# pqh22/ProxyTransformation

Hardware: AMD Instinct MI355X
Metric: scenes/sec (100k pts, 256 clusters, 64 proxies) (higher is better)
Workload: dtype f32; 1 GPU; cfg2: N=100000 pts, gs=8->M'=256 kept clusters, L=64 text + V=196 image proxies, d=256, eval forward; scenes_per_gpu=4, img_feat_dtype=bf16, input_sets_rotated=3, streams=1, lanes=1 (one forward at a time), setup_forwards=32

## Files before the change

include/proxyt.h:

```cpp
#ifndef PROXYT_H_
#define PROXYT_H_

#include <stddef.h>
#include <stdint.h>

#ifdef __cplusplus
extern "C" {
#endif

#define PTX_ABI_VERSION 13

#define PTX_API __attribute__((visibility("default")))

#define PTX_OK          0
#define PTX_EINVAL     -1
#define PTX_ELAUNCH    -2
#define PTX_ENOSPACE   -3
#define PTX_ETIMEOUT   -4
#define PTX_EGATE      -5

typedef struct PtxShape {
    int32_t B;
    int32_t N;
    int32_t grid_size;
// ... 54 lines not shown

PTX_API int         ptx_abi_version(void);
PTX_API const char *ptx_last_error(void);

typedef struct PtxContext PtxContext;
PTX_API int ptx_context_create(PtxContext **ctx);
PTX_API int ptx_context_destroy(PtxContext *ctx);
PTX_API int ptx_context_check(PtxContext *ctx);
PTX_API int ptx_context_sync_check(PtxContext *ctx);
PTX_API int ptx_context_gates(const PtxContext *ctx);

PTX_API int         ptx_kernel_count(void);
PTX_API const char *ptx_kernel_name(int kid);
PTX_API int         ptx_timing_select(int kid);
PTX_API int         ptx_timing_read(int *launches, float *total_ms);
PTX_API int         ptx_timing_every(int n);
PTX_API int         ptx_timing_select_mask(uint64_t mask);
PTX_API int         ptx_timing_read_sites(int *launches, float *total_ms, int n);

PTX_API size_t ptx_prep_bytes(const PtxShape *s);
PTX_API size_t ptx_workspace_bytes(const PtxShape *s);

PTX_API int ptx_workspace_init(const PtxShape *s, void *workspace, size_t ws_bytes, void *stream);

PTX_API int ptx_prepare(const PtxShape *s, const PtxWeights *w, const float *lin,
                void *prep, size_t prep_bytes, void *stream);


PTX_API int ptx_grid_centers(const float *points, int B, int N, const float *lin, int gs, float margin,
                     float *minmax, float *centers, void *workspace, size_t ws_bytes, void *stream);

PTX_API int ptx_ball_query(const float *centers, const float *points, int B, int M, int N, int K,
                   float radius, int32_t *idx, float *cluster, int32_t *pad_count, void *stream);

PTX_API int ptx_linear(const float *x, const float *w, const float *bias, const float *residual, float *y,
               int rows, int n_out, int n_in, int gelu, void *stream);
PTX_API int ptx_linear_ln_partials(const float *x, const float *w, const float *bias, const float *residual, float *y, float *lnp,
               int rows, int n_out, int n_in, void *stream);
PTX_API size_t ptx_ln_linear_scratch_bytes(int n_out, int n_in);
PTX_API int ptx_ln_linear(const float *x, const float *lnp, const float *w, const float *gamma, const float *beta,
               const float *bias, float eps, int gelu, float *y, void *scratch, size_t scratch_bytes,
               int rows, int n_out, int n_in, void *stream);
PTX_API int ptx_gemm_policy(int min_tiles_128);

PTX_API int ptx_offset_net(const PtxShape *s, const PtxWeights *w, const void *prep,
                   const float *centers_in, const float *cluster, const float *minmax,
// ... 248 lines not shown
```

proxytransformation_amd/_abi.py:

```python
from __future__ import annotations

import ctypes as C
import os
from typing import Optional

_HERE = os.path.dirname(os.path.abspath(__file__))
LIB_PATH = os.path.join(_HERE, "libproxyt_hip.so")
ABI_VERSION = 13

c_float_p = C.c_void_p


class PtxShape(C.Structure):
    _fields_ = [(n, C.c_int32) for n in
                ("B", "N", "grid_size", "K", "Mt", "Mk", "L", "V", "C", "heads", "hidden",
                 "in_dim", "hw", "img_dtype")] + \
               [(n, C.c_float) for n in ("radius", "margin", "bn_eps", "ln_eps")]


class PtxSlotMlp(C.Structure):
    _fields_ = [(n, C.c_void_p) for n in ("conv_w", "conv_b", "bn_w", "bn_b", "bn_mean", "bn_var")]


class PtxBlock(C.Structure):
# ... 78 lines not shown
                ("arena_bwd", C.c_void_p), ("arena_bwd_bytes", C.c_size_t), ("grads", C.c_void_p), ("grads_floats", C.c_size_t),
                ("dtext", C.c_void_p), ("dimg", C.c_void_p)]


class PtxForwardOpts(C.Structure):
    _fields_ = [("bbox_enc", C.c_void_p), ("compute_dtype", C.c_int32), ("reserved", C.c_int32 * 5)]


_P, _I, _F, _Z = C.c_void_p, C.c_int, C.c_float, C.c_size_t
_SH, _W = C.POINTER(PtxShape), C.POINTER(PtxWeights)
SIGNATURES = {
    "ptx_abi_version": (C.c_int, []),
    "ptx_last_error": (C.c_char_p, []),
    "ptx_kernel_count": (C.c_int, []),
    "ptx_kernel_name": (C.c_char_p, [_I]),
    "ptx_timing_select": (_I, [_I]),
    "ptx_timing_every": (_I, [_I]),
    "ptx_timing_read": (_I, [C.POINTER(C.c_int), C.POINTER(C.c_float)]),
    "ptx_timing_select_mask": (_I, [C.c_uint64]),
    "ptx_timing_read_sites": (_I, [C.POINTER(C.c_int), C.POINTER(C.c_float), _I]),
    "ptx_prep_bytes": (_Z, [_SH]),
    "ptx_workspace_bytes": (_Z, [_SH]),
    "ptx_workspace_init": (_I, [_SH, _P, _Z, _P]),
    "ptx_prepare": (_I, [_SH, _W, _P, _P, _Z, _P]),
    "ptx_grid_centers": (_I, [_P, _I, _I, _P, _I, _F, _P, _P, _P, _Z, _P]),
    "ptx_ball_query": (_I, [_P, _P, _I, _I, _I, _I, _F, _P, _P, _P, _P]),
    "ptx_linear": (_I, [_P, _P, _P, _P, _P, _I, _I, _I, _I, _P]),
    "ptx_linear_ln_partials": (_I, [_P, _P, _P, _P, _P, _P, _I, _I, _I, _P]),
    "ptx_ln_linear_scratch_bytes": (_Z, [_I, _I]),
    "ptx_ln_linear": (_I, [_P, _P, _P, _P, _P, _P, _F, _I, _P, _P, _Z, _I, _I, _I, _P]),
    "ptx_gemm_policy": (_I, [_I]),
    "ptx_offset_net": (_I, [_SH, _W, _P, _P, _P, _P, _P, _P, _P]),
    "ptx_select_clusters": (_I, [_SH] + [_P] * 14),
    "ptx_pointnet": (_I, [_SH, _W, _P, _P, _P, _P, _P]),
    "ptx_img_proxy": (_I, [_SH, _W, _P, _P, _P, _P, _Z, _P]),
    "ptx_proxy_block": (_I, [_SH, _W, _P, _I, _P, _P, _I, _P, _P, _P, _P, _Z, _P]),
    "ptx_affine_scatter": (_I, [_SH, _P, _P, _P, _P, _P, _P, _P]),
    "ptx_affine_compact": (_I, [_SH, _P, _P, _P, _P, _P, _P, _P, _P, _Z, _P]),
    "ptx_wait_counts": (_I, [_P, _I, C.c_int64]),
    "ptx_context_create": (_I, [C.POINTER(C.c_void_p)]),
    "ptx_context_destroy": (_I, [_P]),
    "ptx_context_check": (_I, [_P]),
    "ptx_context_sync_check": (_I, [_P]),
    "ptx_context_gates": (_I, [_P]),
    "ptx_forward": (_I, [_P, _SH, _W, _P, _P, _P, _P, _P, _P, _P, _P, _P, _P, _P, _P, _Z,
                         C.POINTER(PtxDebug), _P]),
# ... 101 lines not shown
```

proxytransformation_amd/csrc/api.hip:

```cpp
#include <atomic>
#include <chrono>
#include <cmath>
#include <cstdlib>
#include <cstring>
#include <mutex>
#include <utility>
#include <vector>

#include "common.h"

namespace ptx {

static thread_local char g_err[512] = "";

void set_error(const char *fmt, ...)
{
    va_list ap;
    va_start(ap, fmt);
    vsnprintf(g_err, sizeof(g_err), fmt, ap);
    va_end(ap);
}

static const char *const kKernelNames[] = {
    "k_minmax", "k_cluster", "k_select", "k_tags",
// ... 99 lines not shown
    P.posb_t = take((size_t)s.Mk * s.C); P.posb_i = take((size_t)s.Mk * s.C);
    P.w3 = take((size_t)3 * s.C * s.in_dim); P.b3 = take((size_t)3 * s.C);
    P.t1 = take((size_t)s.heads * P.KT1 * P.hd);
    P.t2 = take((size_t)s.heads * P.hd * P.KT2p);
    P.ppg_w = take((size_t)s.C * s.C); P.ppg_c = take(s.C);
    for (int i = 0; i < 2; ++i) {
        P.fc1g_w[i] = take((size_t)s.hidden * s.C); P.fc1g_c[i] = take(s.hidden);
        const size_t planes = mlp_fused_supported(s.C, s.hidden, 1, 0) ? (size_t)s.hidden * s.C * 3 / 2 : 0;
        P.mlp_w1p[i] = take(planes); P.mlp_w2p[i] = take(planes);
    }
    for (int i = 0; i < 2; ++i) P.qkvb[i] = take((size_t)s.Mk * 3 * s.C);
    P.total = o;
    return P;
}

struct LayoutForce { int v[4]; };
static LayoutForce layout_force()
{
    LayoutForce f{{-1, -1, -1, -1}};
    if (const char *e = getenv("PTX_LAYOUT"))
        for (int i = 0; i < 4 && e[i] != '\0'; ++i) f.v[i] = e[i] == '0' ? 0 : (e[i] == '1' ? 1 : -1);
    return f;
}
struct LayoutChoice { double est_cluster, est_image; bool cluster_on_caller, img_late, early; LayoutForce lf; };
static LayoutChoice choose_layout(const PtxShape &S)
{
    static const LayoutForce lf = layout_force();
    LayoutChoice c{};
    c.lf = lf;
    const int B = S.B, Kd = S.Mt - S.Mk;
    const double img_mb = (double)B * S.V * S.in_dim * S.hw * (S.img_dtype == 0 ? 4.0 : 2.0) * 1e-6;
    c.est_cluster = 80.0 + 0.42 * Kd;
    c.est_image = 40.0 + (S.img_dtype == 0 ? 0.98 : 0.78) * img_mb;
    c.cluster_on_caller = lf.v[0] >= 0 ? lf.v[0] != 0 : c.est_cluster > c.est_image + 60.0;
    c.img_late = c.cluster_on_caller && (lf.v[2] >= 0 ? lf.v[2] != 0 : c.est_image + 60.0 < 0.8 * c.est_cluster);
    const double est_all = 1.8 * 12.0 * (double)B * S.Mt * S.C * S.C / 70e6;
    c.early = c.cluster_on_caller && (lf.v[1] >= 0 ? lf.v[1] != 0 : (Kd >= 128 && (long)B * S.Mk >= 1024 && est_all < 3.0 * 0.42 * Kd));
    return c;
}

WsLayout ws_layout(const PtxShape &s)
{
    WsLayout L{};
    const PrepLayout P = prep_layout(s);
    size_t o = 0;
    auto take = [&](size_t bytes) { size_t r = o; o += align_up(bytes, 256); return r; };
    const size_t B = s.B, N = s.N, K = s.K, C = s.C;
    const size_t M = (size_t)s.grid_size * s.grid_size * s.grid_size;
    const size_t Mk = s.Mk, Mt = s.Mt, Kd = s.Mt - s.Mk;
    const size_t nimg = B * s.V, Lp = s.L > s.V ? s.L : s.V, R = B * Mk;
    L.zero_begin = o;
    L.mm_enc = take(B * 6 * 4);
    L.scene_acc = take(B * 2 * 4);
    L.tag = take(B * N * 4);
    L.fa_ticket = take(2 * B * s.heads * 4);
    L.mlp_ticket = take(mlp_ticket_bytes((int)R));
    L.mm_ticket = take(4);
    L.zero_bytes = o - L.zero_begin;
    L.minmax = take(B * 6 * 4);
    L.centers0 = take(B * M * 3 * 4); L.cluster1 = take(B * M * K * 3 * 4);
    L.offsets = take(B * M * 3 * 4);  L.centers = take(B * M * 3 * 4);
    L.idx2 = take(B * M * K * 4);     L.cluster2 = take(B * M * K * 3 * 4);
    L.pad_count = take(B * M * 4);
    L.order = take(B * Mt * 4); L.picks = take(B * (Kd ? Kd : 1) * 4); L.keep = take(B * Mk * 4); L.ksrc = take(B * Mk * 4);
    L.kcenter = take(B * Mk * 3 * 4); L.kcluster = take(B * Mk * K * 3 * 4); L.kidx = take(B * Mk * K * 4);
    L.drop_idx = take(B * (Kd ? Kd : 1) * K * 4);
    L.tile_counts = take(B * (size_t)cdiv(s.N, kTilePts) * 4);
    L.point_proxy = take(R * C * 4);
    for (int i = 0; i < 2; ++i) L.x_in[i] = take(R * C * 4);
    bool may_early = false;
    for (int dt = 0; dt < 3; ++dt) { PtxShape t = s; t.img_dtype = dt; may_early = may_early || choose_layout(t).early; }
    const size_t em = may_early ? 1 : 0;
    L.pp_all = take(em * B * Mt * C * 4); L.order_e = take(em * B * Mt * 4);
    for (int i = 0; i < 2; ++i) { L.xln_all[i] = take(em * B * Mt * C * 4); L.g_all[i] = take(em * B * Mt * 3 * C * 4); }
    L.fm = take(nimg * s.in_dim * 4); L.qkv0 = take(nimg * 3 * C * 4);
    L.we = take(nimg * s.heads * (size_t)P.KT1 * 4);
    {
        const size_t pool_b = img_pool_bytes((int)nimg, s.in_dim, P.KT2p - s.in_dim), gbuf_b = nimg * s.heads * (size_t)P.KT2p * 4;
        L.pool = L.gbuf = take(pool_b > gbuf_b ? pool_b : gbuf_b);
    }
    L.obuf = take(nimg * C * 4); L.cbuf = take(nimg * C * 4); L.img_proxy = take(nimg * C * 4);
    for (int i = 0; i < 2; ++i) {
        L.qkv[i] = take(R * 3 * C * 4); L.pt[i] = take(B * Lp * C * 4); L.pv[i] = take(B * Lp * C * 4);
        L.ao[i] = take(R * C * 4); L.x1[i] = take(R * C * 4); L.xn2[i] = take(0);
        L.hbuf[i] = take(mlp_fused_supported(s.C, s.hidden, (int)R, 0) ? 0 : R * (size_t)s.hidden * 4);
        L.x2[i] = take(R * C * 4); L.guide[i] = take(R * C * 4);
        L.head[i] = take(R * 9 * 4);
        L.lnp_x1[i] = take(R * (C / 32) * 2 * 4);
    }
    L.lnp_img = take(nimg * (C / 32) * 2 * 4);
    const size_t fsp = fattn_split_for(s.B, s.heads);
    L.fa_part = take(fsp > 1 ? 2 * B * s.heads * fsp * Mk * kFaPartRow * 4 : 0);
    L.mlp_part = take(mlp_fused_supported(s.C, s.hidden, (int)R, 0) ? mlp_part_bytes((int)R) : 0);
    L.total = o;
    return L;
}

}
struct PtxContext {
    int dev = -1;
    hipStream_t st = nullptr, lo = nullptr;
    hipEvent_t fork = nullptr, join = nullptr, aux = nullptr, tags = nullptr, early_a = nullptr, early_b = nullptr;
    uint32_t *gate = nullptr; uint32_t gate_seq = 0;
// ... 207 lines not shown
            g.p[0].w2 = prep + P.t1; g.p[0].c2 = we; g.p[0].n2 = P.KT1; g.p[0].ldc2 = s.heads * P.KT1;
            g.p[0].chain_tiles = s.heads; g.p[0].w2_stride = (long)P.KT1 * hd; g.p[0].c2_stride = P.KT1;
        }
        PTX_TIMED(KID_IMG_QKV0, st, launch_gemm(g, st));
    }
    if (!chained) {
        for (int h0 = 0; h0 < s.heads; h0 += kMaxGroups) {
            GemmBatch g{}; g.n = std::min(kMaxGroups, s.heads - h0);
            for (int h = h0; h < h0 + g.n; ++h)
                g.p[h - h0] = GemmProb{qkv0 + h * hd, prep + P.t1 + (size_t)h * P.KT1 * hd, we + (size_t)h * P.KT1,
                                       nullptr, nullptr, nullptr, nullptr, nimg, P.KT1, hd, 3 * C, hd,
                                       s.heads * P.KT1, 0, 0, 0, EPI_NONE};
            PTX_TIMED(KID_IMG_WE, st, launch_gemm(g, st));
        }
    }
    if (pooled32) {
        PTX_TIMED_EXT(KID_IMG_SCORES, st, launch_img_pool32(img, we, qkv0, nimg, s.in_dim, s.hw, C, P.KT1, EW, attn_scale(hd), Gs, E, ML, st));
    } else if (dt == 0) {
        PTX_TIMED(KID_IMG_SCORES, st, launch_img_scores(img, we, qkv0, nimg, s.in_dim, s.hw, s.heads, C, P.KT1,
                                                        P.KT2p, attn_scale(hd), gbuf, st));
        PTX_TIMED(KID_IMG_GATHER, st, launch_img_gather(img, nimg, s.in_dim, s.hw, s.heads, P.KT2p, gbuf, st));
    } else if (pooled) {
        PTX_TIMED_EXT(KID_IMG_SCORES, st, launch_img_pool(img_any, dt, we, qkv0, nimg, s.in_dim, s.hw, C, P.KT1,
                                                      EW, attn_scale(hd), Gs, E, ML, st));
    } else {
        PTX_TIMED(KID_IMG_SCORES, st, launch_img_scores16(img_any, dt, we, qkv0, nimg, s.in_dim, s.hw, s.heads, C,
                                                          P.KT1, P.KT2p, attn_scale(hd), gbuf, st));
        PTX_TIMED(KID_IMG_GATHER, st, launch_img_gather16(img_any, dt, nimg, s.in_dim, s.hw, s.heads, P.KT2p, gbuf, st));
    }
    for (int h0 = 0; h0 < s.heads; h0 += kMaxGroups) {
        GemmBatch g{}; g.n = std::min(kMaxGroups, s.heads - h0);
        for (int h = h0; h < h0 + g.n; ++h) {
            GemmProb &gp = g.p[h - h0];
            gp = GemmProb{gbuf + (size_t)h * P.KT2p, prep + P.t2 + (size_t)h * hd * P.KT2p, obuf + h * hd,
                          w.v_b + h * hd, nullptr, gbuf + (size_t)h * P.KT2p + s.in_dim,
                          qkv0 + 2 * C + h * hd, nimg, hd, P.KT2p, s.heads * P.KT2p, P.KT2p, C,
                          0, s.heads * P.KT2p, 3 * C, EPI_NONE};
            if (pooled) {
                gp.A = nullptr; gp.rs = nullptr;
                gp.pg = Gs + (size_t)h * s.in_dim; gp.ldg = 2 * s.heads * s.in_dim; gp.gslab = s.heads * s.in_dim;
                gp.pe = E + (size_t)h * EW; gp.lde = s.heads * EW;
                gp.pml = ML + (size_t)h * 5; gp.ldml = s.heads * 5;
                gp.kg = s.in_dim;
            }
        }
        PTX_TIMED(KID_IMG_O, st, launch_gemm(g, st));
    }
    {
        GemmBatch g{}; g.n = 1;
        g.p[0] = GemmProb{obuf, w.c_w, cbuf, w.c_b, nullptr, nullptr, nullptr,
                          nimg, C, C, C, C, C, 0, 0, 0, EPI_NONE};
        g.p[0].lnp_out = at<float>(ws, L.lnp_img) + (size_t)i0 * (C / 32) * 2;
        PTX_TIMED(KID_IMG_C, st, launch_gemm(g, st));
    }
    if (need_ln) {
        LnBatch lb{}; lb.n = 1; lb.C = C; lb.eps = s.ln_eps;
        lb.p[0] = LnProb{cbuf, img_proxy, w.norm_img_w, w.norm_img_b, nullptr, nimg, 1};
        PTX_TIMED(KID_IMG_LN, st, launch_ln_rows(lb, st));
    }
    return PTX_OK;
}

struct Branch {
    const PtxBlock *blk; const float *x_in; const float *proxy; int Lp; const uint8_t *mask;
    const float *head_w, *head_b, *head_ab; int nout; float *head_out; float *guide; int slot;
    bool late_proxy;
    const float *proxy_lnp, *pp_gw, *pp_gc;
    const float *fc1_gw, *fc1_gc;
// ... 276 lines not shown
            std::chrono::duration_cast<std::chrono::microseconds>(std::chrono::steady_clock::now() - t0).count() >
                timeout_us)
            return PTX_ETIMEOUT;
    }
}

size_t ptx_prep_bytes(const PtxShape *s)
{
    if (s == nullptr || validate_shape(*s) != PTX_OK) return 0;
    return prep_layout(*s).total * sizeof(float);
}

size_t ptx_workspace_bytes(const PtxShape *s)
{
    if (s == nullptr || validate_shape(*s) != PTX_OK) return 0;
    return ws_layout(*s).total;
}

int ptx_workspace_init(const PtxShape *s, void *workspace, size_t ws_bytes, void *stream)
{
    PTX_TRY(check_bufs(s, workspace, ws_bytes));
    const WsLayout L = ws_layout(*s);
    PTX_HIP(hipMemsetAsync(at<char>(workspace, L.zero_begin), 0, L.zero_bytes, static_cast<hipStream_t>(stream)));
    return PTX_OK;
}

int ptx_prepare(const PtxShape *s, const PtxWeights *w, const float *lin, void *prep, size_t prep_bytes,
                void *stream)
{
    (void)lin;
    PTX_REQUIRE(s && w && prep, "ptx_prepare: null argument");
    PTX_TRY(validate_shape(*s));
    if (prep_bytes < prep_layout(*s).total * sizeof(float)) { set_error("prep buffer too small"); return PTX_ENOSPACE; }
    return run_prepare(*s, *w, static_cast<float *>(prep), static_cast<hipStream_t>(stream));
}

int ptx_grid_centers(const float *points, int B, int N, const float *lin, int gs, float margin,
                     float *minmax, float *centers, void *workspace, size_t ws_bytes, void *stream)
{
    PTX_REQUIRE(points && lin && minmax && centers && workspace, "ptx_grid_centers: null argument");
    PTX_REQUIRE(ws_bytes >= (size_t)B * 6 * 4, "ptx_grid_centers: workspace needs %d bytes", B * 24);
    hipStream_t st = static_cast<hipStream_t>(stream);
    uint32_t *enc = static_cast<uint32_t *>(workspace);
    PTX_HIP(hipMemsetAsync(enc, 0, (size_t)B * 6 * 4, st));
    ScenePts sp;
    PTX_TRY(make_scene_pts(points, nullptr, B, N, &sp));
// ... 315 lines not shown
        float *pp_all = at<float>(ws, L.pp_all), *xa_t = at<float>(ws, L.xln_all[0]), *xa_i = at<float>(ws, L.xln_all[1]);
        int32_t *order_e = at<int32_t>(ws, L.order_e);
        PTX_TRY(launch_order(S, pad_count, order_override, order_e, side->lo));
        PTX_TRY(launch_pointnet(pf + P.enc_ab, w->encoder, centers, cluster2, B * S.Mt, S.Mt, K, S.C, pp_all, &w->text, &w->img, nullptr,
                                nullptr, xa_t, xa_i, S.ln_eps, order_e, M, side->lo, nullptr, 0, true));
        GemmBatch g{}; g.n = 2;
        g.p[0] = GemmProb{xa_t, w->text.qkv_w, at<float>(ws, L.g_all[0]), nullptr, nullptr, nullptr, nullptr, B * S.Mt, 3 * S.C, S.C, S.C, S.C,
                          3 * S.C, 0, 0, 0, EPI_NONE};
        g.p[1] = GemmProb{xa_i, w->img.qkv_w, at<float>(ws, L.g_all[1]), nullptr, nullptr, nullptr, nullptr, B * S.Mt, 3 * S.C, S.C, S.C, S.C,
                          3 * S.C, 0, 0, 0, EPI_NONE};
        PTX_TRY(launch_gemm(g, side->lo, compute_dtype));
        PTX_TRY(run_blocks(S, br, 2, point_proxy, ws, side->lo, 1, compute_dtype, nullptr, nullptr, true));
    }

    int32_t *order = at<int32_t>(ws, L.order), *picks = at<int32_t>(ws, L.picks), *keep = at<int32_t>(ws, L.keep);
    float *kcenter = at<float>(ws, L.kcenter);
    float *kcluster = dbg && debug->kcluster ? at<float>(ws, L.kcluster) : nullptr;
    int32_t *kidx = dbg && debug->kidx ? at<int32_t>(ws, L.kidx) : nullptr;
    int32_t *drop_idx = dbg && debug->drop_idx ? at<int32_t>(ws, L.drop_idx) : nullptr;
    int32_t *ksrc = at<int32_t>(ws, L.ksrc);
    const bool ext_event = !capturing;
    const bool tags_gated = gated && side->lo_ok && (lf.v[3] >= 0 ? lf.v[3] != 0 : est_image < 1.6 * est_cluster);
    const bool tags_tail = !cluster_on_caller && !tags_gated;
    PTX_TIMED(KID_SELECT, cs, launch_select_order(S, centers, pad_count, order_override, order, picks, keep, kcenter,
                                                  ksrc, bbox_in ? nullptr : mm_ws, cs, cluster_on_caller, ext_event && !tags_tail ? side->aux : nullptr,
                                                  cg_join_select ? &cjoin : nullptr));
    int32_t *tile_counts = at<int32_t>(ws, L.tile_counts);
    hipStream_t ts = tags_tail ? cs : side->lo;
    const bool slots_first = !cluster_on_caller && !tags_tail;
    auto enqueue_tags = [&]() -> int {
        if (tags_gated) {
            PTX_TIMED(KID_GATE_TAGS, ts, launch_gate(KID_GATE_TAGS, ts, gate_ref(side, 36, side->gate_seq, 6)));
        } else if (!tags_tail) {
            if (!ext_event) PTX_HIP(hipEventRecord(side->aux, cs));
            PTX_HIP(hipStreamWaitEvent(ts, side->aux, 0));
        }
        if (kcluster || kidx || drop_idx)
            PTX_TRY(launch_select_slots(S, idx2, cluster2, order, picks, keep, kcluster, kidx, drop_idx, nullptr, ts));
        PTX_TIMED(KID_TAGS, ts, launch_tags(S, idx2, order, picks, ksrc, tag, tile_counts, counts, at<int32_t>(ws, L.scene_acc), ts));
        if (tags_gated) {
            auto sig = [&]() -> int {
                hipLaunchKernelGGL(k_signal, dim3(1), dim3(64), 0, ts, side->gate + 38, side->gate_seq);
                PTX_LAUNCHED("k_signal[tags]");
                return PTX_OK;
            };
            PTX_TIMED(KID_SIGNAL_TAGS, ts, sig());
        } else if (cgate) {
            if (!fault_ctags) {
                hipLaunchKernelGGL(k_signal, dim3(1), dim3(64), 0, ts, side->gate + 56, side->gate_seq);
                PTX_LAUNCHED("k_signal[ctags]");
            }
        } else if (!tags_tail) PTX_HIP(hipEventRecord(side->tags, ts));
        return PTX_OK;
    };
    if (slots_first) PTX_TRY(enqueue_tags());

    const bool want_img_proxy = debug != nullptr && debug->img_proxy != nullptr;
// ... 101 lines not shown
```

proxytransformation_amd/csrc/common.h:

```cpp
#pragma once
#include <hip/hip_runtime.h>
#include <cstdarg>
#include <cstdint>
#include <cstdio>

#include "../../include/proxyt.h"

namespace ptx {

void set_error(const char *fmt, ...);
bool timing_ext_take(hipEvent_t *start, hipEvent_t *stop);

#define PTX_REQUIRE(cond, ...)                                   \
    do {                                                         \
        if (!(cond)) {                                           \
            ::ptx::set_error(__VA_ARGS__);                       \
            return PTX_EINVAL;                                   \
        }                                                        \
    } while (0)

#define PTX_HIP(expr)                                                              \
    do {                                                                           \
        hipError_t e_ = (expr);                                                    \
        if (e_ != hipSuccess) {                                                    \
// ... 164 lines not shown
    size_t off_ab, enc_ab;
    size_t ttn_ab, itn_ab;
    size_t posb_t, posb_i;
    size_t w3, b3;
    size_t t1;
    size_t t2;
    size_t ppg_w, ppg_c;
    size_t fc1g_w[2], fc1g_c[2];
    size_t mlp_w1p[2], mlp_w2p[2];
    size_t qkvb[2];
    size_t total;
    int KT1, KT2p, hd;
};
PrepLayout prep_layout(const PtxShape &s);

struct WsLayout {
    size_t zero_begin, zero_bytes;
    size_t mm_enc;
    size_t scene_acc;
    size_t tag;
    size_t fa_ticket;
    size_t mlp_ticket;
    size_t mm_ticket;
    size_t minmax, centers0, cluster1, offsets, centers, idx2, cluster2, pad_count;
    size_t order, picks, keep, ksrc, kcenter, kcluster, kidx, drop_idx, tile_counts;
    size_t point_proxy, x_in[2];
    size_t pp_all, xln_all[2], g_all[2];
    size_t order_e;
    size_t fm, qkv0, we, pool, gbuf, obuf, cbuf, img_proxy;
    size_t qkv[2], pt[2], pv[2], ao[2], x1[2], xn2[2], hbuf[2], x2[2], guide[2], head[2];
    size_t lnp_img, lnp_x1[2];
    size_t fa_part;
    size_t mlp_part;
    size_t total;
};
WsLayout ws_layout(const PtxShape &s);

int validate_shape(const PtxShape &s);

enum : int { EPI_NONE = 0, EPI_GELU = 1 };
struct GemmProb {
    const float *A; const float *W; float *C;
    const float *bias;
    const float *res;
    const float *rs;
    const float *ad;
    int R, N, K, lda, ldw, ldc, ldres, rs_stride, ldad, epi;
    const float *pg, *pe, *pml; int ldg, gslab, lde, ldml, kg;
    float *lnp_out;
    const float *lnp_in, *ln_c; int ln_parts, ln_C; float ln_eps;
    const float *w2; float *c2; int n2, ldc2, chain_tiles; long w2_stride, c2_stride;
};
constexpr int kMaxGroups = 8;
struct GemmBatch {
    GemmProb p[kMaxGroups]; int n; int rotate;
    GateRef tail_gate;
};
int launch_gemm(const GemmBatch &gb, hipStream_t st, int compute_dtype = 0);
int gemm_policy(int min_tiles_128);

struct LnProb { const float *x; float *y; const float *w; const float *b; const float *add; int R, add_rows; };
struct LnBatch { LnProb p[2]; int n; int C; float eps; };
int launch_ln_rows(const LnBatch &lb, hipStream_t st);

struct HeadProb {
    const float *x; const float *nw; const float *nb;
    const float *hw; const float *hb;
    const float *ab;
    float *out; float *guide; int R, nout;
};
struct HeadBatch { HeadProb p[2]; int n; int C; float eps; };
int launch_heads(const HeadBatch &hb, hipStream_t st);

struct AttnProb {
    const float *Q, *K, *V; float *O; const uint8_t *mask;
    int nq, nk, ldq, ldk, ldv, ldo;
    long sQ, sK, sV, sO;
};
// ... 72 lines not shown
int launch_affine(const PtxShape &s, const ScenePts &points, uint32_t *tag, const float *kcenter,
                  const float *translate, const float *transform, float *out, int32_t *counts,
                  const int32_t *tile_counts, bool compact, bool clear_tag, hipStream_t st,
                  const uint32_t *poison = nullptr);

int launch_img_mean(const float *img, int nimg, int in_dim, int hw, float *fm, hipStream_t st,
                    uint32_t *gate = nullptr, uint32_t gate_seq = 0);
int launch_img_scores(const float *img, const float *we, const float *qkv0, int nimg, int in_dim,
                      int hw, int heads, int C, int KT1, int KT2p, float scale, float *gbuf,
                      hipStream_t st);
int launch_img_gather(const float *img, int nimg, int in_dim, int hw, int heads, int KT2p,
                      float *gbuf, hipStream_t st);

int launch_img_mean16(const void *img, int dt, int nimg, int in_dim, int hw, float *fm, hipStream_t st,
                      uint32_t *gate = nullptr, uint32_t gate_seq = 0);
int launch_img_scores16(const void *img, int dt, const float *we, const float *qkv0, int nimg, int in_dim,
                        int hw, int heads, int C, int KT1, int KT2p, float scale, float *gbuf, hipStream_t st);
int launch_img_gather16(const void *img, int dt, int nimg, int in_dim, int hw, int heads, int KT2p, float *gbuf,
                        hipStream_t st);
bool img_pool_supported(int dt, int in_dim, int hw, int heads);
size_t img_pool_bytes(int nimg, int in_dim, int EW);
void img_pool_layout(float *scratch, int nimg, int in_dim, int EW, float **Gs, float **E, float **ML);
int launch_img_pool(const void *img, int dt, const float *we, const float *qkv0, int nimg, int in_dim, int hw, int C,
                    int KT1, int EW, float scale, float *Gs, float *E, float *ML, hipStream_t st);

bool img_pool32_supported(int dt, int in_dim, int hw, int heads);
int launch_img_pool32(const float *img, const float *we, const float *qkv0, int nimg, int in_dim, int hw, int C, int KT1, int EW,
                      float scale, float *Gs, float *E, float *ML, hipStream_t st);

int run_prepare(const PtxShape &s, const PtxWeights &w, float *prep, hipStream_t st);

}
```

proxytransformation_amd/csrc/gemm.hip:

```cpp
#include <atomic>
#include <cstdlib>

#include "common.h"
#include "split3.h"

namespace ptx {

constexpr int BK = 32, LDT = BK + 4;

__device__ __forceinline__ void pin4(float4 &v) { asm volatile("" : "+v"(v.x), "+v"(v.y), "+v"(v.z), "+v"(v.w)); }
__device__ __forceinline__ void ln_row_stats(const GemmProb &pr, int row, float &mu, float &rstd)
{
    const float2 *pp = reinterpret_cast<const float2 *>(pr.lnp_in) + (size_t)row * pr.ln_parts;
    constexpr int kMaxParts = 16;
    float2 v[kMaxParts];
#pragma unroll
    for (int t = 0; t < kMaxParts; ++t) v[t] = pp[min(t, pr.ln_parts - 1)];
    float s1 = 0.0f, s2 = 0.0f;
#pragma unroll
    for (int t = 0; t < kMaxParts; ++t) { s1 += t < pr.ln_parts ? v[t].x : 0.0f; s2 += t < pr.ln_parts ? v[t].y : 0.0f; }
    const float inv = 1.0f / (float)pr.ln_C;
    mu = s1 * inv;
    float between = 0.0f;
#pragma unroll
// ... 755 lines not shown
        PTX_REQUIRE(p.lnp_in == nullptr || (p.ln_c && p.ln_parts >= 1 && p.ln_parts <= 16 && p.ln_C == 32 * p.ln_parts &&
                                            p.K == p.ln_C && p.pg == nullptr && p.bias == nullptr),
                    "gemm: bad LayerNorm-consumer description in group %d", g);
        any_ln = any_ln || p.lnp_in != nullptr;
        rmax = p.R > rmax ? p.R : rmax;
        nmax = p.N > nmax ? p.N : nmax;
        kmin = p.K < kmin ? p.K : kmin;
        kmax = p.K > kmax ? p.K : kmax;
        tiles32 += (long)cdiv(p.R, 32) * cdiv(p.N, 32);
    }
    if (gb.p[0].w2 != nullptr) {
        PTX_REQUIRE(gb.n == 1 && gb.p[0].pg == nullptr && gb.p[0].c2 && gb.p[0].n2 >= 1 && gb.p[0].chain_tiles >= 1 &&
                    gb.p[0].chain_tiles * 32 <= gb.p[0].N && gb.p[0].K >= 4 * BK && gb.p[0].lnp_out == nullptr && !any_ln,
                    "gemm: bad chained-product description");
        PTX_TRY((launch_gemm32<4, 0, true>(gb, rmax, nmax, st)));
        PTX_LAUNCHED("k_gemm");
        return PTX_OK;
    }
    constexpr int g64_min = 1024;
    long tiles128 = 0;
    for (int g = 0; g < gb.n; ++g) tiles128 += (long)cdiv(gb.p[g].R, 128) * cdiv(gb.p[g].N, 128);
    const int min128 = g_gemm128_min_tiles.load(std::memory_order_relaxed);
    const bool enough = tiles128 >= min128 && (min128 == 1 || 2 * tiles128 >= 3 * (long)min128 || kmin >= 512);
    const bool use128 = gb.p[0].pg == nullptr && kmin == kmax && kmin % 256 == 0 && kmin <= 4096 && min128 > 0 && enough;
    if (use128) {
        const dim3 grid(cdiv(rmax, 128), cdiv(nmax, 128), gb.n);
        const int nrep = kmin / (32 * PTX_G128_NM);
        if (compute_dtype == 1) {
            if (any_ln) hipLaunchKernelGGL((k_gemm128x<PTX_G128_NM, 1, true>), grid, dim3(256), 0, st, gb, nrep);
            else        hipLaunchKernelGGL((k_gemm128x<PTX_G128_NM, 1>), grid, dim3(256), 0, st, gb, nrep);
        } else {
            if (any_ln) hipLaunchKernelGGL((k_gemm128x<PTX_G128_NM, 3, true>), grid, dim3(256), 0, st, gb, nrep);
            else        hipLaunchKernelGGL((k_gemm128x<PTX_G128_NM, 3>), grid, dim3(256), 0, st, gb, nrep);
        }
        PTX_LAUNCHED("k_gemm128x");
        return PTX_OK;
    }
    if (compute_dtype == 1 && gb.p[0].pg == nullptr && kmin == kmax && kmin % 128 == 0 && kmin / 128 <= 8) {
        const dim3 grid(cdiv(rmax, 64), cdiv(nmax, 64), gb.n);
        const int nkg = kmin / 128;
        if (any_ln && nkg == 1) hipLaunchKernelGGL((k_gemm64x<1, 1, 1, true>), grid, dim3(256), 0, st, gb);
        else if (any_ln && nkg == 2) hipLaunchKernelGGL((k_gemm64x<2, 1, 1, true>), grid, dim3(256), 0, st, gb);
        else if (any_ln && nkg == 4) hipLaunchKernelGGL((k_gemm64x<4, 1, 1, true>), grid, dim3(256), 0, st, gb);
        else if (any_ln) { set_error("gemm: LayerNorm consumer with K=%d in bf16 mode", kmin); return PTX_EINVAL; }
        else if (nkg == 1) hipLaunchKernelGGL((k_gemm64x<1, 1, 1>), grid, dim3(256), 0, st, gb);
        else if (nkg == 2) hipLaunchKernelGGL((k_gemm64x<2, 1, 1>), grid, dim3(256), 0, st, gb);
        else if (nkg == 4) hipLaunchKernelGGL((k_gemm64x<4, 1, 1>), grid, dim3(256), 0, st, gb);
        else if (nkg == 8) hipLaunchKernelGGL((k_gemm64x<8, 1, 1>), grid, dim3(256), 0, st, gb);
        else if (nkg == 6) hipLaunchKernelGGL((k_gemm64x<2, 3, 1>), grid, dim3(256), 0, st, gb);
        else { set_error("gemm: K=%d in bf16 mode", kmin); return PTX_EINVAL; }
        PTX_LAUNCHED("k_gemm64x<bf16>");
        return PTX_OK;
    }
    if (gb.p[0].pg != nullptr) {
        PTX_TRY((launch_gemm32<4, 1>(gb, rmax, nmax, st)));
    } else if (tiles32 >= g64_min) {
        const dim3 grid(cdiv(rmax, 64), cdiv(nmax, 64), gb.n);
        const int nkg = (kmin == kmax && kmin % 128 == 0) ? kmin / 128 : 0;
        if (any_ln && nkg == 1) hipLaunchKernelGGL((k_gemm64x<1, 1, 3, true>), grid, dim3(256), 0, st, gb);
        else if (any_ln && nkg == 2) hipLaunchKernelGGL((k_gemm64x<2, 1, 3, true>), grid, dim3(256), 0, st, gb);
        else if (any_ln && nkg == 4) hipLaunchKernelGGL((k_gemm64x<4, 1, 3, true>), grid, dim3(256), 0, st, gb);
        else if (any_ln) hipLaunchKernelGGL(k_gemm64<true>, grid, dim3(256), 0, st, gb);
        else if (nkg == 1) hipLaunchKernelGGL((k_gemm64x<1, 1>), grid, dim3(256), 0, st, gb);
        else if (nkg == 2) hipLaunchKernelGGL((k_gemm64x<2, 1>), grid, dim3(256), 0, st, gb);
        else if (nkg == 4) hipLaunchKernelGGL((k_gemm64x<4, 1>), grid, dim3(256), 0, st, gb);
        else if (nkg == 8) hipLaunchKernelGGL((k_gemm64x<8, 1>), grid, dim3(256), 0, st, gb);
        else if (nkg == 6) hipLaunchKernelGGL((k_gemm64x<2, 3>), grid, dim3(256), 0, st, gb);
        else if (nkg == 12) hipLaunchKernelGGL((k_gemm64x<4, 3>), grid, dim3(256), 0, st, gb);
        else if (nkg == 16) hipLaunchKernelGGL((k_gemm64x<8, 2>), grid, dim3(256), 0, st, gb);
        else if (nkg == 32) hipLaunchKernelGGL((k_gemm64x<8, 4>), grid, dim3(256), 0, st, gb);
        else hipLaunchKernelGGL(k_gemm64<false>, grid, dim3(256), 0, st, gb);
    } else {
        const int nk = cdiv(kmin, BK);
        int sk = 1;
        while (sk < 4 && tiles32 * sk < 4096 && nk >= 4 * sk) sk *= 2;
        if (any_ln) {
            if (sk == 1) PTX_TRY((launch_gemm32<1, 0, false, true>(gb, rmax, nmax, st)));
            else if (sk == 2) PTX_TRY((launch_gemm32<2, 0, false, true>(gb, rmax, nmax, st)));
// ... 139 lines not shown
```

proxytransformation_amd/csrc/imgpool.hip:

```cpp
#include <cstdlib>
#include <hip/hip_ext.h>

#include "common.h"

namespace ptx {

typedef unsigned int u4u2 __attribute__((ext_vector_type(4), aligned(2)));
typedef unsigned int u32x4 __attribute__((ext_vector_type(4)));
typedef float f32x4 __attribute__((ext_vector_type(4)));
typedef __bf16 bf16x8 __attribute__((ext_vector_type(8)));

constexpr int kPoolHeads = 8;
constexpr int kPoolNtImages = 4096;
constexpr int kPoolWPad = 544;
constexpr int kPoolPPad = 136;

typedef _Float16 f16x8 __attribute__((ext_vector_type(8)));

template <int DT>
__device__ __forceinline__ void split3(float x, unsigned short &q1, unsigned short &q2, unsigned short &q3)
{
    if (DT == 1) {
        const unsigned int u1 = __float_as_uint(x) & 0xffff0000u;
        const float r1 = x - __uint_as_float(u1);
// ... 29 lines not shown
__device__ __forceinline__ u32x4 shr_elems(const u32x4 &v, int k)
{
    const int ws = k >> 1;
    unsigned int w[8] = {v[0], v[1], v[2], v[3], 0u, 0u, 0u, 0u};
    u32x4 o;
#pragma unroll
    for (int q = 0; q < 4; ++q) {
        unsigned int lo = 0u, hi = 0u;
#pragma unroll
        for (int s = 0; s < 4; ++s) {
            if (ws == s) { lo = w[q + s]; hi = w[q + s + 1]; }
        }
        o[q] = (k & 1) ? ((lo >> 16) | (hi << 16)) : lo;
    }
    return o;
}

struct PoolArgs {
    const unsigned short *img; const float *we, *qkv0;
    int nimg, in_dim, hw, C, KT1, EW; float scale;
    float *Gs;
    float *E;
    float *ML;
};

template <int DT, bool NT>
__global__ __launch_bounds__(512) void k_img_pool(PoolArgs a)
{
    constexpr int heads = kPoolHeads;
    extern __shared__ __attribute__((aligned(16))) unsigned char smem[];
    float *partial = reinterpret_cast<float *>(smem);
    unsigned short *wpart = reinterpret_cast<unsigned short *>(partial + 8 * heads * 128);
    unsigned short *parts = wpart + 24 * kPoolWPad;
    const int in_dim = a.in_dim, hw = a.hw;
    const int xcd = blockIdx.x & 7, slot = blockIdx.x >> 3;
    const int T = slot & 1, imr = (slot >> 1) * 8 + xcd;
    if (imr >= a.nimg) return;
    const int im = a.nimg - 1 - imr;
    const int slab = im * 2 + T;
    const int tid = threadIdx.x, lane = lane_id();
    const int wid = __builtin_amdgcn_readfirstlane(tid >> 6);
    const int n = lane & 15, kq = lane >> 4;
    const float *wim = a.we + (size_t)im * heads * a.KT1;
    const unsigned short *f = a.img + (size_t)im * in_dim * hw;
    const int px = 128 * T + 8 * n;
    const bool full = px + 8 <= hw;
    const int cw = 64 * wid;
// ... 85 lines not shown
    }
    __syncthreads();

    {
        const int h = wid;
        float e[2], mloc = -INFINITY, sv[2];
#pragma unroll
        for (int u = 0; u < 2; ++u) {
            const int p = lane + 64 * u;
            float s = 0.0f;
#pragma unroll
            for (int w = 0; w < 8; ++w) s += partial[((size_t)w * heads + h) * 128 + p];
            sv[u] = 128 * T + p < hw ? s + ev[u] : -INFINITY;
            mloc = fmaxf(mloc, sv[u]);
        }
        const float m = wave_max(mloc);
#pragma unroll
        for (int u = 0; u < 2; ++u) e[u] = 128 * T + lane + 64 * u < hw ? expf(sv[u] - m) : 0.0f;
        const float l = wave_sum(e[0] + e[1]);
        float *erow = a.E + ((size_t)im * heads + h) * a.EW;
        const float s0 = T == 0 ? wave_sum(sq * sk) * a.scale : 0.0f;
        if (lane == 0) {
            float *ml = a.ML + ((size_t)im * heads + h) * 5;
            ml[2 * T] = m;
            ml[2 * T + 1] = l;
            if (T == 0) { ml[4] = s0; erow[0] = 1.0f; }
        }
#pragma unroll
        for (int u = 0; u < 2; ++u) {
            const int p = lane + 64 * u;
            const int t = 1 + 128 * T + p;
            if (t <= hw || (T == (hw > 128 ? 1 : 0) && t < a.EW)) erow[t] = t <= hw ? e[u] : 0.0f;
            unsigned short q1, q2, q3;
            split3<DT>(DT == 2 ? e[u] * kPoolEScale : e[u], q1, q2, q3);
            parts[(size_t)h * kPoolPPad + p] = q1;
            parts[(size_t)(8 + h) * kPoolPPad + p] = q2;
            parts[(size_t)(16 + h) * kPoolPPad + p] = q3;
        }
    }
    __syncthreads();

    {
        const int ps = n & 3, hh = n >> 2;
        const int src = ((ps + 4 * kq) + 16 * (n >> 2)) * 4;
        u32x4 bfr[2][3];
#pragma unroll
        for (int hg = 0; hg < 2; ++hg)
#pragma unroll
            for (int pt = 0; pt < 3; ++pt)
                bfr[hg][pt] = *reinterpret_cast<const u32x4 *>(parts + (size_t)(pt * 8 + 4 * hg + hh) * kPoolPPad + 8 * (ps + 4 * kq));
        const unsigned m0 = ps == 0 ? ~0u : 0u, m1 = ps == 1 ? ~0u : 0u, m2 = ps == 2 ? ~0u : 0u, m3 = ps == 3 ? ~0u : 0u;
        float *G = partial;
#pragma unroll
        for (int kb = 0; kb < 2; ++kb) {
#pragma unroll
// ... 27 lines not shown
                    }
            }
            if (ps == 0) {
#pragma unroll
                for (int hg = 0; hg < 2; ++hg)
#pragma unroll
                    for (int q = 0; q < 2; ++q)
                        *reinterpret_cast<f32x4 *>(G + (size_t)(4 * hg + hh) * in_dim + cw + 32 * kb + 8 * kq + 4 * q) =
                            f32x4{xs[hg][4 * q], xs[hg][4 * q + 1], xs[hg][4 * q + 2], xs[hg][4 * q + 3]};
            }
        }
    }
    __syncthreads();
    {
        const float *G = partial;
        float *dst = a.Gs + (size_t)slab * heads * in_dim;
        for (int i = tid * 4; i < heads * in_dim; i += 512 * 4)
        {
            const f32x4 v = *reinterpret_cast<const f32x4 *>(G + i);
            if (NT) asm volatile("global_store_dwordx4 %0, %1, off sc1 nt" :: "v"(dst + i), "v"(v) : "memory");
            else    asm volatile("global_store_dwordx4 %0, %1, off sc1" :: "v"(dst + i), "v"(v) : "memory");
        }
    }
}

bool img_pool_supported(int dt, int in_dim, int hw, int heads)
{
    return (dt == 1 || dt == 2) && heads == kPoolHeads && in_dim == 512 && hw > 128 && hw <= 255;
}

size_t img_pool_bytes(int nimg, int in_dim, int EW)
{
    return (size_t)nimg * kPoolHeads * (2 * (size_t)in_dim + EW + 8) * sizeof(float);
}

void img_pool_layout(float *scratch, int nimg, int in_dim, int EW, float **Gs, float **E, float **ML)
{
    *Gs = scratch;
    *E = *Gs + (size_t)nimg * 2 * kPoolHeads * in_dim;
    *ML = *E + (size_t)nimg * kPoolHeads * EW;
}

int launch_img_pool(const void *img, int dt, const float *we, const float *qkv0, int nimg, int in_dim, int hw, int C,
                    int KT1, int EW, float scale, float *Gs, float *E, float *ML, hipStream_t st)
{
    PTX_REQUIRE(EW % 4 == 0 && EW >= hw + 1 && hw > 128 && hw <= 255, "img pool: hw=%d EW=%d", hw, EW);
    PoolArgs pa{static_cast<const unsigned short *>(img), we, qkv0, nimg, in_dim, hw, C, KT1, EW, scale, Gs, E, ML};
    const size_t lds = sizeof(float) * 8 * kPoolHeads * 128 + sizeof(unsigned short) * 24 * (kPoolWPad + kPoolPPad);
    PTX_REQUIRE(lds <= 64 * 1024, "img pool: %zu B of LDS", lds);
    static const int nt_env = getenv("PTX_POOL_NT") ? atoi(getenv("PTX_POOL_NT")) : -1;
    const bool nt = nt_env >= 0 ? nt_env != 0 : nimg >= kPoolNtImages;
    const dim3 grid(cdiv(nimg, 8) * 16);
    hipEvent_t ta = nullptr, tb = nullptr;
    (void)timing_ext_take(&ta, &tb);
    if (dt == 1) { if (nt) hipExtLaunchKernelGGL((k_img_pool<1, true>), grid, dim3(512), lds, st, ta, tb, 0, pa); else hipExtLaunchKernelGGL((k_img_pool<1, false>), grid, dim3(512), lds, st, ta, tb, 0, pa); }
    else         { if (nt) hipExtLaunchKernelGGL((k_img_pool<2, true>), grid, dim3(512), lds, st, ta, tb, 0, pa); else hipExtLaunchKernelGGL((k_img_pool<2, false>), grid, dim3(512), lds, st, ta, tb, 0, pa); }
    PTX_LAUNCHED("k_img_pool");
    return PTX_OK;
}

}
```

Before: 18220 scenes/s.

## Merge split-T image pool partials in last-arriving block via tickets

```diff
diff --git a/include/proxyt.h b/include/proxyt.h
--- a/include/proxyt.h
+++ b/include/proxyt.h
@@ -100,6 +100,9 @@
 PTX_API size_t ptx_workspace_bytes(const PtxShape *s);
 
 PTX_API int ptx_workspace_init(const PtxShape *s, void *workspace, size_t ws_bytes, void *stream);
+
+PTX_API int ptx_img_pool_regions(const PtxShape *s, size_t *rows_offset, size_t *rows_bytes, size_t *tickets_offset,
+                                 size_t *tickets_bytes);
 
 PTX_API int ptx_prepare(const PtxShape *s, const PtxWeights *w, const float *lin,
                 void *prep, size_t prep_bytes, void *stream);
diff --git a/proxytransformation_amd/_abi.py b/proxytransformation_amd/_abi.py
--- a/proxytransformation_amd/_abi.py
+++ b/proxytransformation_amd/_abi.py
@@ -124,6 +124,7 @@
     "ptx_prep_bytes": (_Z, [_SH]),
     "ptx_workspace_bytes": (_Z, [_SH]),
     "ptx_workspace_init": (_I, [_SH, _P, _Z, _P]),
+    "ptx_img_pool_regions": (_I, [_SH] + [C.POINTER(C.c_size_t)] * 4),
     "ptx_prepare": (_I, [_SH, _W, _P, _P, _Z, _P]),
     "ptx_grid_centers": (_I, [_P, _I, _I, _P, _I, _F, _P, _P, _P, _Z, _P]),
     "ptx_ball_query": (_I, [_P, _P, _I, _I, _I, _I, _F, _P, _P, _P, _P]),
diff --git a/proxytransformation_amd/csrc/api.hip b/proxytransformation_amd/csrc/api.hip
--- a/proxytransformation_amd/csrc/api.hip
+++ b/proxytransformation_amd/csrc/api.hip
@@ -145,6 +145,7 @@
         for (int i = 0; i < 4 && e[i] != '\0'; ++i) f.v[i] = e[i] == '0' ? 0 : (e[i] == '1' ? 1 : -1);
     return f;
 }
+constexpr size_t kPoolRowsGuard = 256;
 struct LayoutChoice { double est_cluster, est_image; bool cluster_on_caller, img_late, early; LayoutForce lf; };
 static LayoutChoice choose_layout(const PtxShape &S)
 {
@@ -179,6 +180,7 @@
     L.fa_ticket = take(2 * B * s.heads * 4);
     L.mlp_ticket = take(mlp_ticket_bytes((int)R));
     L.mm_ticket = take(4);
+    L.pool_ticket = take(nimg * 4);
     L.zero_bytes = o - L.zero_begin;
     L.minmax = take(B * 6 * 4);
     L.centers0 = take(B * M * 3 * 4); L.cluster1 = take(B * M * K * 3 * 4);
@@ -198,10 +200,8 @@
     for (int i = 0; i < 2; ++i) { L.xln_all[i] = take(em * B * Mt * C * 4); L.g_all[i] = take(em * B * Mt * 3 * C * 4); }
     L.fm = take(nimg * s.in_dim * 4); L.qkv0 = take(nimg * 3 * C * 4);
     L.we = take(nimg * s.heads * (size_t)P.KT1 * 4);
-    {
-        const size_t pool_b = img_pool_bytes((int)nimg, s.in_dim, P.KT2p - s.in_dim), gbuf_b = nimg * s.heads * (size_t)P.KT2p * 4;
-        L.pool = L.gbuf = take(pool_b > gbuf_b ? pool_b : gbuf_b);
-    }
+    L.pool = take(img_pool_bytes((int)nimg, s.in_dim, P.KT2p - s.in_dim));
+    L.gbuf = take(nimg * s.heads * (size_t)P.KT2p * 4 + kPoolRowsGuard);
     L.obuf = take(nimg * C * 4); L.cbuf = take(nimg * C * 4); L.img_proxy = take(nimg * C * 4);
     for (int i = 0; i < 2; ++i) {
         L.qkv[i] = take(R * 3 * C * 4); L.pt[i] = take(B * Lp * C * 4); L.pv[i] = take(B * Lp * C * 4);
@@ -455,7 +455,7 @@
         PTX_TIMED(KID_IMG_GATHER, st, launch_img_gather(img, nimg, s.in_dim, s.hw, s.heads, P.KT2p, gbuf, st));
     } else if (pooled) {
         PTX_TIMED_EXT(KID_IMG_SCORES, st, launch_img_pool(img_any, dt, we, qkv0, nimg, s.in_dim, s.hw, C, P.KT1,
-                                                      EW, attn_scale(hd), Gs, E, ML, st));
+                                                      EW, attn_scale(hd), Gs, E, ML, gbuf, P.KT2p, at<int>(ws, L.pool_ticket) + i0, st));
     } else {
         PTX_TIMED(KID_IMG_SCORES, st, launch_img_scores16(img_any, dt, we, qkv0, nimg, s.in_dim, s.hw, s.heads, C,
                                                           P.KT1, P.KT2p, attn_scale(hd), gbuf, st));
@@ -469,7 +469,7 @@
                           w.v_b + h * hd, nullptr, gbuf + (size_t)h * P.KT2p + s.in_dim,
                           qkv0 + 2 * C + h * hd, nimg, hd, P.KT2p, s.heads * P.KT2p, P.KT2p, C,
                           0, s.heads * P.KT2p, 3 * C, EPI_NONE};
-            if (pooled) {
+            if (pooled32) {
                 gp.A = nullptr; gp.rs = nullptr;
                 gp.pg = Gs + (size_t)h * s.in_dim; gp.ldg = 2 * s.heads * s.in_dim; gp.gslab = s.heads * s.in_dim;
                 gp.pe = E + (size_t)h * EW; gp.lde = s.heads * EW;
@@ -477,6 +477,7 @@
                 gp.kg = s.in_dim;
             }
         }
+        g.sliced32 = pooled && !pooled32;
         PTX_TIMED(KID_IMG_O, st, launch_gemm(g, st));
     }
     {
@@ -799,6 +800,18 @@
     PTX_TRY(check_bufs(s, workspace, ws_bytes));
     const WsLayout L = ws_layout(*s);
     PTX_HIP(hipMemsetAsync(at<char>(workspace, L.zero_begin), 0, L.zero_bytes, static_cast<hipStream_t>(stream)));
+    return PTX_OK;
+}
+
+int ptx_img_pool_regions(const PtxShape *s, size_t *rows_offset, size_t *rows_bytes, size_t *tickets_offset, size_t *tickets_bytes)
+{
+    PTX_REQUIRE(s && rows_offset && rows_bytes && tickets_offset && tickets_bytes, "ptx_img_pool_regions: null argument");
+    PTX_TRY(validate_shape(*s));
+    const WsLayout L = ws_layout(*s);
+    const PrepLayout P = prep_layout(*s);
+    const size_t nimg = (size_t)s->B * s->V;
+    *rows_offset = L.gbuf; *rows_bytes = nimg * s->heads * (size_t)P.KT2p * 4;
+    *tickets_offset = L.pool_ticket; *tickets_bytes = nimg * 4;
     return PTX_OK;
 }
 
@@ -1160,8 +1173,9 @@
     const bool ext_event = !capturing;
     const bool tags_gated = gated && side->lo_ok && (lf.v[3] >= 0 ? lf.v[3] != 0 : est_image < 1.6 * est_cluster);
     const bool tags_tail = !cluster_on_caller && !tags_gated;
+    const bool select_event = ext_event && !tags_tail && !tags_gated;
     PTX_TIMED(KID_SELECT, cs, launch_select_order(S, centers, pad_count, order_override, order, picks, keep, kcenter,
-                                                  ksrc, bbox_in ? nullptr : mm_ws, cs, cluster_on_caller, ext_event && !tags_tail ? side->aux : nullptr,
+                                                  ksrc, bbox_in ? nullptr : mm_ws, cs, cluster_on_caller, select_event ? side->aux : nullptr,
                                                   cg_join_select ? &cjoin : nullptr));
     int32_t *tile_counts = at<int32_t>(ws, L.tile_counts);
     hipStream_t ts = tags_tail ? cs : side->lo;
@@ -1170,7 +1184,7 @@
         if (tags_gated) {
             PTX_TIMED(KID_GATE_TAGS, ts, launch_gate(KID_GATE_TAGS, ts, gate_ref(side, 36, side->gate_seq, 6)));
         } else if (!tags_tail) {
-            if (!ext_event) PTX_HIP(hipEventRecord(side->aux, cs));
+            if (!select_event) PTX_HIP(hipEventRecord(side->aux, cs));
             PTX_HIP(hipStreamWaitEvent(ts, side->aux, 0));
         }
         if (kcluster || kidx || drop_idx)
diff --git a/proxytransformation_amd/csrc/common.h b/proxytransformation_amd/csrc/common.h
--- a/proxytransformation_amd/csrc/common.h
+++ b/proxytransformation_amd/csrc/common.h
@@ -210,6 +210,7 @@
     size_t fa_ticket;
     size_t mlp_ticket;
     size_t mm_ticket;
+    size_t pool_ticket;
     size_t minmax, centers0, cluster1, offsets, centers, idx2, cluster2, pad_count;
     size_t order, picks, keep, ksrc, kcenter, kcluster, kidx, drop_idx, tile_counts;
     size_t point_proxy, x_in[2];
@@ -242,6 +243,7 @@
 constexpr int kMaxGroups = 8;
 struct GemmBatch {
     GemmProb p[kMaxGroups]; int n; int rotate;
+    int sliced32;
     GateRef tail_gate;
 };
 int launch_gemm(const GemmBatch &gb, hipStream_t st, int compute_dtype = 0);
@@ -360,7 +362,7 @@
 size_t img_pool_bytes(int nimg, int in_dim, int EW);
 void img_pool_layout(float *scratch, int nimg, int in_dim, int EW, float **Gs, float **E, float **ML);
 int launch_img_pool(const void *img, int dt, const float *we, const float *qkv0, int nimg, int in_dim, int hw, int C,
-                    int KT1, int EW, float scale, float *Gs, float *E, float *ML, hipStream_t st);
+                    int KT1, int EW, float scale, float *Gs, float *E, float *ML, float *rows, int ldrow, int *tickets, hipStream_t st);
 
 bool img_pool32_supported(int dt, int in_dim, int hw, int heads);
 int launch_img_pool32(const float *img, const float *we, const float *qkv0, int nimg, int in_dim, int hw, int C, int KT1, int EW,
diff --git a/proxytransformation_amd/csrc/gemm.hip b/proxytransformation_amd/csrc/gemm.hip
--- a/proxytransformation_amd/csrc/gemm.hip
+++ b/proxytransformation_amd/csrc/gemm.hip
@@ -801,7 +801,7 @@
     for (int g = 0; g < gb.n; ++g) tiles128 += (long)cdiv(gb.p[g].R, 128) * cdiv(gb.p[g].N, 128);
     const int min128 = g_gemm128_min_tiles.load(std::memory_order_relaxed);
     const bool enough = tiles128 >= min128 && (min128 == 1 || 2 * tiles128 >= 3 * (long)min128 || kmin >= 512);
-    const bool use128 = gb.p[0].pg == nullptr && kmin == kmax && kmin % 256 == 0 && kmin <= 4096 && min128 > 0 && enough;
+    const bool use128 = gb.p[0].pg == nullptr && !gb.sliced32 && kmin == kmax && kmin % 256 == 0 && kmin <= 4096 && min128 > 0 && enough;
     if (use128) {
         const dim3 grid(cdiv(rmax, 128), cdiv(nmax, 128), gb.n);
         const int nrep = kmin / (32 * PTX_G128_NM);
@@ -815,7 +815,7 @@
         PTX_LAUNCHED("k_gemm128x");
         return PTX_OK;
     }
-    if (compute_dtype == 1 && gb.p[0].pg == nullptr && kmin == kmax && kmin % 128 == 0 && kmin / 128 <= 8) {
+    if (compute_dtype == 1 && gb.p[0].pg == nullptr && !gb.sliced32 && kmin == kmax && kmin % 128 == 0 && kmin / 128 <= 8) {
         const dim3 grid(cdiv(rmax, 64), cdiv(nmax, 64), gb.n);
         const int nkg = kmin / 128;
         if (any_ln && nkg == 1) hipLaunchKernelGGL((k_gemm64x<1, 1, 1, true>), grid, dim3(256), 0, st, gb);
@@ -833,6 +833,9 @@
     }
     if (gb.p[0].pg != nullptr) {
         PTX_TRY((launch_gemm32<4, 1>(gb, rmax, nmax, st)));
+    } else if (gb.sliced32) {
+        PTX_REQUIRE(!any_ln && kmin >= 4 * BK, "gemm: sliced32 with K=%d", kmin);
+        PTX_TRY((launch_gemm32<4, 0>(gb, rmax, nmax, st)));
     } else if (tiles32 >= g64_min) {
         const dim3 grid(cdiv(rmax, 64), cdiv(nmax, 64), gb.n);
         const int nkg = (kmin == kmax && kmin % 128 == 0) ? kmin / 128 : 0;
diff --git a/proxytransformation_amd/csrc/imgpool.hip b/proxytransformation_amd/csrc/imgpool.hip
--- a/proxytransformation_amd/csrc/imgpool.hip
+++ b/proxytransformation_amd/csrc/imgpool.hip
@@ -75,7 +75,23 @@
     float *Gs;
     float *E;
     float *ML;
+    float *rows;
+    int *tickets;
+    int ldrow;
 };
+
+__device__ __forceinline__ void pool_st_agent(float *p, float v) { __hip_atomic_store(p, v, __ATOMIC_RELAXED, __HIP_MEMORY_SCOPE_AGENT); }
+__device__ __forceinline__ float pool_ld_agent(const float *p) { return __hip_atomic_load(p, __ATOMIC_RELAXED, __HIP_MEMORY_SCOPE_AGENT); }
+__device__ __forceinline__ f32x4 pool_ld4_agent(const float *p)
+{
+    f32x4 v;
+    asm volatile("global_load_dwordx4 %0, %1, off sc1" : "=v"(v) : "v"(p) : "memory");
+    return v;
+}
+__device__ __forceinline__ void pool_wait_agent(f32x4 &a, f32x4 &b)
+{
+    asm volatile("s_waitcnt vmcnt(0)" : "+v"(a), "+v"(b) :: "memory");
+}
 
 template <int DT, bool NT>
 __global__ __launch_bounds__(512) void k_img_pool(PoolArgs a)
@@ -207,15 +223,15 @@
         const float s0 = T == 0 ? wave_sum(sq * sk) * a.scale : 0.0f;
         if (lane == 0) {
             float *ml = a.ML + ((size_t)im * heads + h) * 5;
-            ml[2 * T] = m;
-            ml[2 * T + 1] = l;
-            if (T == 0) { ml[4] = s0; erow[0] = 1.0f; }
+            pool_st_agent(ml + 2 * T, m);
+            pool_st_agent(ml + 2 * T + 1, l);
+            if (T == 0) { pool_st_agent(ml + 4, s0); pool_st_agent(erow, 1.0f); }
         }
 #pragma unroll
         for (int u = 0; u < 2; ++u) {
             const int p = lane + 64 * u;
             const int t = 1 + 128 * T + p;
-            if (t <= hw || (T == (hw > 128 ? 1 : 0) && t < a.EW)) erow[t] = t <= hw ? e[u] : 0.0f;
+            if (t <= hw || (T == (hw > 128 ? 1 : 0) && t < a.EW)) pool_st_agent(erow + t, t <= hw ? e[u] : 0.0f);
             unsigned short q1, q2, q3;
             split3<DT>(DT == 2 ? e[u] * kPoolEScale : e[u], q1, q2, q3);
             parts[(size_t)h * kPoolPPad + p] = q1;
@@ -289,6 +305,48 @@
             else    asm volatile("global_store_dwordx4 %0, %1, off sc1" :: "v"(dst + i), "v"(v) : "memory");
         }
     }
+    asm volatile("s_waitcnt vmcnt(0)" ::: "memory");
+    __syncthreads();
+    int *flag = reinterpret_cast<int *>(wpart);
+    if (tid == 0) flag[0] = __hip_atomic_fetch_add(a.tickets + im, 1, __ATOMIC_RELAXED, __HIP_MEMORY_SCOPE_AGENT);
+    __syncthreads();
+    if (flag[0] != 1) return;
+    if (tid == 0) __hip_atomic_store(a.tickets + im, 0, __ATOMIC_RELAXED, __HIP_MEMORY_SCOPE_AGENT);
+    {
+        const int h = wid;
+        const float *own = partial + (size_t)h * in_dim;
+        const float *oth = a.Gs + ((size_t)(im * 2 + (1 - T)) * heads + h) * in_dim;
+        const float *ml = a.ML + ((size_t)im * heads + h) * 5;
+        const float *erow = a.E + ((size_t)im * heads + h) * a.EW;
+        float *row = a.rows + ((size_t)im * heads + h) * a.ldrow;
+        f32x4 pv[2];
+#pragma unroll
+        for (int u = 0; u < 2; ++u) pv[u] = pool_ld4_agent(oth + 4 * lane + 256 * u);
+        const float m0 = pool_ld_agent(ml), l0 = pool_ld_agent(ml + 1), m1 = pool_ld_agent(ml + 2), l1 = pool_ld_agent(ml + 3);
+        const float s0 = pool_ld_agent(ml + 4);
+        float et[4];
+#pragma unroll
+        for (int u = 0; u < 4; ++u) et[u] = lane + 64 * u < a.EW ? pool_ld_agent(erow + lane + 64 * u) : 0.0f;
+        pool_wait_agent(pv[0], pv[1]);
+        const float m = fmaxf(fmaxf(m0, m1), s0);
+        const float x0 = __expf(m0 - m), x1 = __expf(m1 - m), xt = __expf(s0 - m);
+        const float inv = 1.0f / ((l0 * x0 + l1 * x1) + xt);
+        const float fc0 = x0 * inv, fc1 = x1 * inv, fct = xt * inv;
+#pragma unroll
+        for (int u = 0; u < 2; ++u) {
+            const f32x4 mine = *reinterpret_cast<const f32x4 *>(own + 4 * lane + 256 * u);
+            const f32x4 g0 = T == 0 ? mine : pv[u], g1 = T == 0 ? pv[u] : mine;
+            const f32x4 v = {g0[0] * fc0 + g1[0] * fc1, g0[1] * fc0 + g1[1] * fc1, g0[2] * fc0 + g1[2] * fc1, g0[3] * fc0 + g1[3] * fc1};
+            float *dst = row + 4 * lane + 256 * u;
+            if (NT) asm volatile("global_store_dwordx4 %0, %1, off sc1 nt" :: "v"(dst), "v"(v) : "memory");
+            else    asm volatile("global_store_dwordx4 %0, %1, off sc1" :: "v"(dst), "v"(v) : "memory");
+        }
+#pragma unroll
+        for (int u = 0; u < 4; ++u) {
+            const int t = lane + 64 * u;
+            if (t < a.EW) pool_st_agent(row + in_dim + t, et[u] * (t == 0 ? fct : (t <= 128 ? fc0 : fc1)));
+        }
+    }
 }
 
 bool img_pool_supported(int dt, int in_dim, int hw, int heads)
@@ -309,10 +367,11 @@
 }
 
 int launch_img_pool(const void *img, int dt, const float *we, const float *qkv0, int nimg, int in_dim, int hw, int C,
-                    int KT1, int EW, float scale, float *Gs, float *E, float *ML, hipStream_t st)
-{
-    PTX_REQUIRE(EW % 4 == 0 && EW >= hw + 1 && hw > 128 && hw <= 255, "img pool: hw=%d EW=%d", hw, EW);
-    PoolArgs pa{static_cast<const unsigned short *>(img), we, qkv0, nimg, in_dim, hw, C, KT1, EW, scale, Gs, E, ML};
+                    int KT1, int EW, float scale, float *Gs, float *E, float *ML, float *rows, int ldrow, int *tickets, hipStream_t st)
+{
+    PTX_REQUIRE(EW % 4 == 0 && EW >= hw + 1 && EW <= 256 && hw > 128 && hw <= 255, "img pool: hw=%d EW=%d", hw, EW);
+    PTX_REQUIRE(rows && tickets && ldrow >= in_dim + EW && ldrow % 4 == 0 && in_dim == 512, "img pool: bad merged-row description");
+    PoolArgs pa{static_cast<const unsigned short *>(img), we, qkv0, nimg, in_dim, hw, C, KT1, EW, scale, Gs, E, ML, rows, tickets, ldrow};
     const size_t lds = sizeof(float) * 8 * kPoolHeads * 128 + sizeof(unsigned short) * 24 * (kPoolWPad + kPoolPPad);
     PTX_REQUIRE(lds <= 64 * 1024, "img pool: %zu B of LDS", lds);
     static const int nt_env = getenv("PTX_POOL_NT") ? atoi(getenv("PTX_POOL_NT")) : -1;
```

Result: slower. 17400 scenes/s (-4.5%).
